# mym-br/gama_tts

Hardware: AMD Instinct MI355X
Metric: audio samples/sec (whole node), batched VTM @44.1kHz (higher is better)
Workload: dtype f32

## Files before the change

### gama_tts_amd/capi.py

```python
import ctypes
import os

import numpy as np

_HERE = os.path.dirname(os.path.abspath(__file__))
_LIB_NAME = "libgama_vtm.so"
N_PARAM = 16
DEVICE_NONE = -1
PRECISION_F64 = 0
PRECISION_MIXED = 1
PRECISION_F32 = 2
TUBE_10_6 = 0
TUBE_30_18 = 1
TABLE_FIR, TABLE_SRC_H, TABLE_SRC_DH, TABLE_WAVETABLE = 0, 1, 2, 3
_STATUS_UNSUPPORTED = 4


class GvtmError(RuntimeError):
    def __init__(self, status, message):
        super().__init__("gvtm status %d: %s" % (status, message))
        self.status = status


class Config(ctypes.Structure):
# ... 171 lines not shown
    if hasattr(L, "gvtm_plan_create_model5_float"):
        L.gvtm_plan_create_model5_float.argtypes = [ctypes.POINTER(Config5), dbl, i32, ctypes.POINTER(vp)]
        L.gvtm_plan_create_model5_float.restype = i32
    L.gvtm_plan_set_timing.argtypes = [vp, i32]
    L.gvtm_plan_set_timing.restype = i32
    L.gvtm_plan_take_kernel_ms.argtypes = [vp, ctypes.POINTER(i32)]
    L.gvtm_plan_take_kernel_ms.restype = dbl
    if diagnostics:
        L.gvtm_debug_set_rows.argtypes = [vp, i32]
        L.gvtm_debug_set_rows.restype = i32
        L.gvtm_debug_set_taps.argtypes = [vp, vp]
        L.gvtm_debug_set_phase_cycles.argtypes = [vp, vp]
        L.gvtm_debug_dpp_selftest.argtypes = [vp, vp]
        L.gvtm_debug_short_math.argtypes = [i32, vp, sz, vp]
        L.gvtm_debug_device_float_math.argtypes = [vp, i32, vp, sz, vp]
        L.gvtm_debug_group_voices.argtypes = [vp, vp, sz, i32, vp, vp, vp, vp]
        L.gvtm_debug_group_voices.restype = i32
    _libs[diagnostics] = L
    return L


def device_count():
    return int(load_library().gvtm_device_count())


class PinnedArray:

    def __init__(self, shape, dtype):
        self._lib = load_library()
        self.array = None
# ... 413 lines not shown
```

### gama_tts_amd/csrc/vtm_capi.cpp

```cpp
#include <hip/hip_runtime.h>

#include <algorithm>
#include <cstdlib>
#include <cstring>
#include <memory>
#include <new>
#include <string>
#include <utility>
#include <vector>

#include "../../include/gama_vtm.h"
#include "vtm_design.hpp"
#include "vtm_kernels.hpp"
#include "vtm_tracks.hpp"
#include "vtm_math.hpp"

namespace {

thread_local std::string g_last_error;

int fail(int status, const std::string& msg)
{
	g_last_error = msg;
	return status;
// ... 73 lines not shown
};

}

#ifndef GVTM_NOISE_TABLE
#define GVTM_NOISE_TABLE 1
#endif

struct gvtm_plan {
	std::vector<gvtm::Design> designs;
	int device = 0;
	int precision = GVTM_PRECISION_F64;
	int rows = 0;
	DeviceBuffer d_wavetable, d_fir, d_src_h, d_src_dh;
	DeviceBuffer d_consts, d_consts5;
	DeviceBuffer d_noise;
	size_t noise_len = 0;
	std::vector<DeviceBuffer> noise_retired;
	struct {
		DeviceBuffer params, frames, audio, counts, maxabs, pcm, scales, voice_ids, groups;
	} host;
	struct {
		DeviceBuffer params, frames, groups;
	} async;
	std::vector<gvtm::TrackConstants> voice_tracks;
	DeviceBuffer d_voice_tracks;
	int compute_units = 0;
	bool timing = false;
	double* debug_taps = nullptr;
	unsigned long long* phase_cycles = nullptr;
// ... 64 lines not shown
	plan->device = device;
	hipDeviceProp_t prop;
	if ((e = hipGetDeviceProperties(&prop, device)) != hipSuccess) return fail_hip(e, "hipGetDeviceProperties");
	if (std::strncmp(prop.gcnArchName, "gfx950", 6) != 0) {
		return fail(GVTM_ERR_NO_DEVICE, std::string("kernels are built for gfx950 only, device is ") + prop.gcnArchName);
	}
	plan->compute_units = prop.multiProcessorCount;
	return GVTM_OK;
}

int upload_tables(gvtm_plan* plan)
{
	const gvtm::Design& dg = plan->designs[0];
	std::vector<gvtm::DeviceConstants> consts;
	std::vector<gvtm::Model5Constants> consts5;
	std::vector<double> wavetables;
	std::vector<float> wavetables_f;
	for (const gvtm::Design& dv : plan->designs) {
		consts.push_back(dv.k);
		if (dg.model5) consts5.push_back(dv.k5);
		wavetables.insert(wavetables.end(), dv.wavetable.begin(), dv.wavetable.end());
		wavetables_f.insert(wavetables_f.end(), dv.wavetable_f.begin(), dv.wavetable_f.end());
	}
	auto upload_design = [&](DeviceBuffer& dst, const std::vector<double>& wide, const std::vector<float>& narrow) {
		return dg.f32 ? upload(dst, narrow) : upload(dst, wide);
	};
	hipError_t e;
	if (!dg.model5) {
		if ((e = upload_design(plan->d_wavetable, wavetables, wavetables_f)) != hipSuccess) return fail_hip(e, "upload wavetable");
		if ((e = upload_design(plan->d_fir, dg.fir, dg.fir_f)) != hipSuccess) return fail_hip(e, "upload fir");
	}
	if ((e = upload_design(plan->d_src_h, dg.src_h, dg.src_h_f)) != hipSuccess) return fail_hip(e, "upload src_h");
	if ((e = upload_design(plan->d_src_dh, dg.src_dh, dg.src_dh_f)) != hipSuccess) return fail_hip(e, "upload src_dh");
	if ((e = upload(plan->d_consts, consts)) != hipSuccess) return fail_hip(e, "upload constants");
	if (dg.model5 && (e = upload(plan->d_consts5, consts5)) != hipSuccess) return fail_hip(e, "upload model 5 constants");
	return GVTM_OK;
}

template <typename Config, typename Differs>
int create_plan(const Config* configs, size_t n_voices, double control_rate, int device, gvtm_plan** plan_out, const char* shared_keys,
		Differs differs, std::string (*design)(const Config&, double, gvtm::Design&))
{
	if (!configs || !plan_out) return fail(GVTM_ERR_INVALID_ARGUMENT, "null config or plan_out");
	*plan_out = nullptr;
	if (n_voices == 0) return fail(GVTM_ERR_INVALID_ARGUMENT, "a plan needs at least one voice");
	if (n_voices > 0x7fffffffu) return fail(GVTM_ERR_INVALID_ARGUMENT, "too many voices");
	for (size_t v = 1; v < n_voices; ++v) {
		if (differs(configs[0], configs[v])) {
			return fail(GVTM_ERR_INVALID_ARGUMENT, "voice " + std::to_string(v) + ": " + shared_keys + " must be those of voice 0 "
					"(one plan is one model at one output rate)");
// ... 269 lines not shown
		case 2: out[i] = gvtm::vmath::cos_short(x[i]); break;
		case 3: out[i] = gvtm::vmath::tan_short(x[i]); break;
		case 4: out[i] = gvtm::vmath::powf_base2(static_cast<float>(x[i])); break;
		case 5: out[i] = gvtm::vmath::powf_base10(static_cast<float>(x[i])); break;
		case 6: out[i] = gvtm::vmath::cosf_glibc(static_cast<float>(x[i])); break;
		case 7: out[i] = gvtm::vmath::tanf_glibc(static_cast<float>(x[i])); break;
		case 8: out[i] = gvtm::vmath::sinf_glibc(static_cast<float>(x[i])); break;
		default: return GVTM_ERR_INVALID_ARGUMENT;
		}
	}
	return GVTM_OK;
}

int gvtm_debug_device_float_math(gvtm_plan* plan, int kind, const float* x, size_t n, float* out)
{
	if (!plan || !x || !out || kind < 0 || kind > 5) return fail(GVTM_ERR_INVALID_ARGUMENT, "bad argument");
	if (plan->device == GVTM_DEVICE_NONE) return fail(GVTM_ERR_NO_DEVICE, "design-only plan");
	DeviceScope scope(plan->device);
	hipError_t e = scope.status();
	if (e != hipSuccess) return fail_hip(e, "hipSetDevice");
	DeviceBuffer dx, dout;
	if ((e = dx.ensure(n * sizeof(float))) != hipSuccess) return fail_hip(e, "hipMalloc");
	if ((e = dout.ensure(n * sizeof(float))) != hipSuccess) return fail_hip(e, "hipMalloc");
	e = hipMemcpy(dx.ptr, x, n * sizeof(float), hipMemcpyHostToDevice);
	if (e == hipSuccess) e = gvtm::launch_float_math_probe(kind, static_cast<const float*>(dx.ptr), n, static_cast<float*>(dout.ptr), nullptr);
	if (e == hipSuccess) e = hipMemcpy(out, dout.ptr, n * sizeof(float), hipMemcpyDeviceToHost);
	if (e != hipSuccess) return fail_hip(e, "float math probe");
	return GVTM_OK;
}

int gvtm_debug_group_voices(gvtm_plan* plan, const int32_t* d_voice_ids, size_t batch, int rows, int32_t* d_row_map, int32_t* d_group_voice,
		int64_t* d_out_counts, float* d_maxabs)
{
	if (!plan || !d_voice_ids || !d_row_map || !d_group_voice || batch == 0 || rows < 1) return fail(GVTM_ERR_INVALID_ARGUMENT, "bad argument");
	if (plan->device == GVTM_DEVICE_NONE) return fail(GVTM_ERR_NO_DEVICE, "design-only plan");
	DeviceScope scope(plan->device);
	hipError_t e = scope.status();
	if (e != hipSuccess) return fail_hip(e, "hipSetDevice");
	DeviceBuffer counts;
	if ((e = counts.ensure(sizeof(int32_t) * plan->n_voices() * gvtm::kGroupVoicesThreads)) != hipSuccess) return fail_hip(e, "hipMalloc");
	const size_t groups = (batch + rows - 1) / rows + static_cast<size_t>(plan->n_voices());
	gvtm::GroupVoicesArgs ga{d_voice_ids, batch, plan->n_voices(), rows, groups, d_row_map, d_group_voice, static_cast<int32_t*>(counts.ptr), d_out_counts, d_maxabs};
// ... 182 lines not shown
	}
	args.src_h = plan->d_src_h.ptr;
	args.src_dh = plan->d_src_dh.ptr;
	args.max_frames = r.max_frames;
	args.audio_stride = r.audio_stride;
	args.batch = r.batch;
	if (r.sl) {
		args.stream = r.sl->d_state;
		args.stream_stride = r.sl->stride;
		args.stream_mode = r.sl->mode;
		if (r.voices && !dg.model5) args.stream_chunk = gvtm::synth_chunk_length(dg.k, plan->precision, 1);
	}
	args.debug_taps = r.voices ? nullptr : plan->debug_taps;
	args.phase_cycles = r.voices ? nullptr : plan->phase_cycles;
	args.k5const = static_cast<const gvtm::Model5Constants*>(plan->d_consts5.ptr);
	return args;
}

template <typename Launch>
int timed_launch(gvtm_plan* plan, hipStream_t stream, const char* what, Launch launch)
{
	hipError_t e;
	EventPair ev;
	if (plan->timing) {
		if (!plan->pool.empty()) {
			ev = std::move(plan->pool.back());
			plan->pool.pop_back();
		} else {
			if ((e = hipEventCreate(&ev.start.h)) != hipSuccess) return fail_hip(e, "hipEventCreate");
			if ((e = hipEventCreate(&ev.stop.h)) != hipSuccess) return fail_hip(e, "hipEventCreate");
// ... 786 lines not shown
```

### gama_tts_amd/csrc/vtm_design.hpp

```cpp
#pragma once

#include <cstddef>
#include <cstdint>
#include <string>
#include <vector>

#include "../../include/gama_vtm.h"

namespace gvtm {

constexpr int kWavetableLength = 512;
constexpr int kSrcZeroCrossings = 13;
constexpr int kSrcPhases = 256;
constexpr int kSrcFilterLength = kSrcZeroCrossings * kSrcPhases;
constexpr int kSrcRing = 1024;
constexpr int kMaxFirTaps = 64;
constexpr int kMaxSectionDelay = 4;
constexpr int kMaxPad = 96;

struct DeviceConstants {
	int sample_rate;
	unsigned control_steps;
	float interp_coef;
	int section_delay;
// ... 9 lines not shown
	double damping;
	double radius_coef[8];
	double aperture_radius2;
	double nasal_r2_sq;
	double nasal_k[6];
	double mouth_b0_refl, mouth_a1_refl, mouth_a_rad;
	double nose_b0_refl, nose_a1_refl, nose_a_rad;
	double throat_b0, throat_a1, throat_gain;
	double bp_T;
	int upsampling;
	int pad;
	unsigned time_inc;
	unsigned phase_inc;
	double src_ratio;
};

struct Model5Constants {
	double sample_rate;
	double output_rate;
	int bypass, constant_mouth;
	double rb_t1, rb_tn_min, rb_tn_max;
	double gn_b0, gn_a1;
	double gp_b0, gp_a1;
	double fn_b0, fn_b1, fn_a1, fn_a2;
	double frication_factor;
	double min_loss, max_loss;
	double nasal_r1_sq;
	double nasal_k[6];
	double period;
	double nose_c[6];
// ... 86 lines not shown
```

### gama_tts_amd/csrc/vtm_device_common.inc

```
#pragma once


constexpr int kDppRowShr1 = 0x111;
constexpr int kDppRowShl1 = 0x101;

__device__ __forceinline__ float from_left(float v)
{
	return __int_as_float(__builtin_amdgcn_update_dpp(0, __float_as_int(v), kDppRowShr1, 0xF, 0xF, true));
}
__device__ __forceinline__ float from_right(float v)
{
	return __int_as_float(__builtin_amdgcn_update_dpp(0, __float_as_int(v), kDppRowShl1, 0xF, 0xF, true));
}
__device__ __forceinline__ double from_left(double v)
{
	const int lo = __builtin_amdgcn_update_dpp(0, __double2loint(v), kDppRowShr1, 0xF, 0xF, true);
	const int hi = __builtin_amdgcn_update_dpp(0, __double2hiint(v), kDppRowShr1, 0xF, 0xF, true);
	return __hiloint2double(hi, lo);
}
__device__ __forceinline__ double from_right(double v)
{
	const int lo = __builtin_amdgcn_update_dpp(0, __double2loint(v), kDppRowShl1, 0xF, 0xF, true);
	const int hi = __builtin_amdgcn_update_dpp(0, __double2hiint(v), kDppRowShl1, 0xF, 0xF, true);
	return __hiloint2double(hi, lo);
// ... 85 lines not shown

__device__ __forceinline__ double frequency_dev(double pitch)
{
	return 220.0 * vmath::exp2_short((pitch + 3.0) * (1.0 / 12.0));
}
__device__ __forceinline__ float frequency_dev(float pitch)
{
	const float x = rmul(pitch + 3.0f, static_cast<float>(1.0 / 12.0));
	return rmul(220.0f, vmath::powf_base2(x));
}

__device__ __forceinline__ double tan_dev(double t) { return vmath::tan_short(t); }
__device__ __forceinline__ double cos_dev(double t) { return vmath::cos_short(t); }
__device__ __forceinline__ float tan_dev(float t) { return vmath::tanf_glibc(t); }
__device__ __forceinline__ float cos_dev(float t) { return vmath::cosf_glibc(t); }

template <typename T> struct Pair;
template <> struct Pair<double> { using type = double2; };
template <> struct Pair<float> { using type = float2; };

__device__ __forceinline__ double noise_advance(double seed)
{
#pragma clang fp contract(off)
	const double product = seed * 377.0;
	return product - floor(product);
}

__device__ __forceinline__ float fdiv_n(float a, float b)
{
	float r = __builtin_amdgcn_rcpf(b);
// ... 50 lines not shown
```

### gama_tts_amd/csrc/vtm_diag_kernels.hip

```cpp
#include <hip/hip_runtime.h>

#include <cstdint>

#include "vtm_design.hpp"
#include "vtm_kernels.hpp"
#include "vtm_math.hpp"

namespace gvtm {

namespace {
#include "vtm_device_common.inc"
}

__global__ void dpp_selftest_kernel(int* out)
{
	const int lane = threadIdx.x & 63;
	const double v = static_cast<double>(lane);
	out[lane] = static_cast<int>(from_left(v));
	out[64 + lane] = static_cast<int>(from_right(v));
	out[128 + lane] = static_cast<int>(row_rotate<6>(v));
	out[192 + lane] = static_cast<int>(row_rotate<10>(v));
	out[256 + lane] = static_cast<int>(from_left_wave(v));
	out[320 + lane] = static_cast<int>(from_right_wave(v));
	out[384 + lane] = static_cast<int>(row_bcast<3>(v));
// ... 3 lines not shown
}


hipError_t launch_dpp_selftest(int* d_out, hipStream_t stream)
{
	hipLaunchKernelGGL(dpp_selftest_kernel, dim3(1), dim3(64), 0, stream, d_out);
	return hipGetLastError();
}

__global__ void float_math_probe_kernel(int kind, const float* x, size_t n, float* out)
{
	const size_t i = static_cast<size_t>(blockIdx.x) * blockDim.x + threadIdx.x;
	if (i >= n) return;
	const float v = x[i];
	float r = 0.0f;
	switch (kind) {
	case 0: r = frequency_dev(v); break;
	case 1: r = amplitude_60db_dev(v); break;
	case 2: r = tan_dev(v); break;
	case 3: r = cos_dev(v); break;
	case 4: r = fdiv_n(v, x[i ^ 1]); break;
	case 5: r = vmath::sinf_glibc(v); break;
	}
	out[i] = r;
}

hipError_t launch_float_math_probe(int kind, const float* d_x, size_t n, float* d_out, hipStream_t stream)
{
	hipLaunchKernelGGL(float_math_probe_kernel, dim3(static_cast<unsigned>((n + 255) / 256)), dim3(256), 0, stream, kind, d_x, n, d_out);
	return hipGetLastError();
// ... 4 lines not shown
```

### gama_tts_amd/csrc/vtm_kernel_v2.inc

```

namespace v2 {

namespace {

constexpr int kPrm = 17;
constexpr int kF1Planes = 6;
constexpr int kF1U = 0, kF1Sig = 1, kF1Thr = 2, kF1B0 = 3, kF1A1 = 4, kF1A2 = 5;
constexpr int kKl = 11;
constexpr int kKlK8 = 7, kKlNk1 = 8, kKlAlr = 9, kKlAu = 10;
constexpr int kInj = 9;
template <typename CT, int LAYOUT>
constexpr bool lane_rec()
{
	return sizeof(CT) == 4 && LAYOUT == 0;
}
constexpr int kLrZero = 16, kLrAlr = 17, kLrAu = 18, kLrK8 = 19, kLrKn = 20, kLrInj = 21, kLrLen = 31;
constexpr int kl_len(bool lr)
{
	return lr ? kLrLen : kKl;
}
template <typename CT>
constexpr bool fr_compact()
{
	return sizeof(CT) == 8;
// ... 405 lines not shown
	__syncthreads();

	if (a.stream) {
		for (int u = 0; u < U; ++u) {
			if (GVTM_ROW_UTT(u, group * U + u) >= a.batch) break;
			const unsigned char* sb = a.stream + GVTM_ROW_UTT(u, (group * U + u)) * a.stream_stride;
			const ST* ring = reinterpret_cast<const ST*>(sb + SL::ring(kTubeLanes, kTubeWords));
			for (int i = tid; i < XRS; i += kThreads) sm.x[u * XRS + i] = ring[i < XR ? i : i - XR];
			const CT* pre = reinterpret_cast<const CT*>(sb + SL::wpre(kTubeLanes, kTubeWords));
			for (int i = tid; i < kWPre; i += kThreads) sm.w[static_cast<size_t>(u) * (kWPre + 2 * C) + i] = pre[i];
		}
		__syncthreads();
	}

	const DeviceConstants& k = *sm.kc;
	int max_chunks = 0;
#pragma unroll
	for (int u = 0; u < U; ++u) max_chunks = sm.ext[u].nchunks > max_chunks ? sm.ext[u].nchunks : max_chunks;

	auto valid_in = [&](int u, int c) -> int {
		const Extent e = sm.ext[u];
		if (c < 0 || c >= e.nchunks) return -1;
		const uint32_t left = e.steps - static_cast<uint32_t>(c) * C;
		return left < static_cast<uint32_t>(C) ? static_cast<int>(left) : C;
	};

	constexpr bool kRowView = !TL::kWaveWide || U > 1;
	const int L = kRowView ? (lane & 15) : lane;
	const int row = kRowView ? (lane >> 4) : 0;
	constexpr bool kTubePerWave = TL::kWaveWide && U > 1;
	constexpr int kFirstHelper = kTubePerWave ? kSerial : 5 * G;
	const int role = kTubePerWave ? (wave < U ? 0 : (wave < kSerial ? wave - U + 1 : 5)) : (wave < 5 * G ? wave / G : 5);
	const int sub = kTubePerWave ? (wave < U ? wave : 0) : (wave < 5 * G ? wave % G : 0);
	const int urow = (U >= 4) ? sub * 4 + row : row % U;
	constexpr int kState = (2 * D + 1) > 5 ? (2 * D + 1) : 5;
	CT st[kState];
#pragma unroll
	for (int i = 0; i < kState; ++i) st[i] = CT(0.0);
	CT& sc_pos = st[0];
// ... 54 lines not shown

	unsigned long long role_busy = 0;
#if GVTM_TUNE_TRACE
	int tr_n = 0;
	auto TR = [&](int t, unsigned id) {
		if (a.phase_cycles != nullptr && group == 0 && lane == 0 && t >= GVTM_TUNE_TRACE && t < GVTM_TUNE_TRACE + 2 && tr_n < 128)
			a.phase_cycles[32768 + wave * 128 + tr_n++] = (static_cast<unsigned long long>(id) << 48) | (clock64() & 0xFFFFFFFFFFFFull);
	};
#else
	auto TR = [](int, unsigned) {};
#endif
	const bool stamping = a.phase_cycles != nullptr && lane == 0;


	auto stage_p2a = [&](int c, int pass) {
		for (int item = pass * 64 + hl; item < U * C && item < (pass + 1) * 64; item += 64) {
			const int u = item / C, s = item - u * C;
			if (s >= valid_in(u, c)) continue;
			const float* pv = sm.prm + at_prm(c & 1, u) + s * kPrm;
			const CT pitch = pv[0], gv = pv[1], av = pv[2];
			const CT f0 = frequency_dev(pitch);
			sm.inc[((c & 1) * U + u) * C + s] = (f0 / CT(2.0)) * CT(k.basic_increment);
			sm.amp[amp_at(c & 3, u, 0, s)] = amplitude_60db_dev(gv);
			sm.amp[amp_at(c & 3, u, 1, s)] = amplitude_60db_dev(av);
		}
	};

	constexpr int kP4aItems = 1;
	auto stage_p4a = [&](int c, int pass) {
		if constexpr (U == 1) {
// ... 51 lines not shown
			const CT v = wl[q] + rmul(p[q] - static_cast<CT>(lower[q]), wu[q] - wl[q]);
			CT* slot = sm.w + (static_cast<size_t>(c % 3) * U + u[q]) * (kWPre + 2 * C);
			slot[kWPre + h[q]] = v;
			if (GVTM_KERNEL_TAPS && a.debug_taps) {
				a.debug_taps[(GVTM_ROW_UTT(u[q], (group * U + u[q])) * a.max_frames * k.control_steps + static_cast<size_t>(c) * C + (h[q] >> 1)) * 8 + 5 + (h[q] & 1)] = p[q];
			}
			if (h[q] >= 2 * C - kWPre) {
				CT* next = sm.w + (static_cast<size_t>((c + 1) % 3) * U + u[q]) * (kWPre + 2 * C);
				next[h[q] - (2 * C - kWPre)] = v;
			}
		}
	};

	auto stage_p4b = [&](int c, int pass) {
		const int taps = k.fir_taps;
		for (int item = pass * 64 + hl; item < U * C && item < (pass + 1) * 64; item += 64) {
			const int u = item / C, s = item - u * C;
			if (s >= valid_in(u, c)) continue;
			CT lp_table = CT(0.0);
			if (kNoiseTable && a.noise_lp != nullptr) lp_table = static_cast<const CT*>(a.noise_lp)[sm.ext[u].step_base + static_cast<unsigned long long>(c) * C + s];
			const CT* wp = sm.w + (static_cast<size_t>(c % 3) * U + u) * (kWPre + 2 * C) + kWPre + 2 * s + 1;
			using CT2 = typename Pair<CT>::type;
			CT acc = 0;
			auto fir_mad = [](CT w, CT cf, CT sum) -> CT {
				if constexpr (sizeof(CT) == 4) return sum + rmul(w, cf);
				else return __builtin_fma(w, cf, sum);
			};
			constexpr int kNT = sizeof(CT) == 8 ? 49 : 47;
			if (sizeof(CT) == 4 && taps == kNT) {
				CT2 wv[kNT / 2];
// ... 33 lines not shown
					}
				}
				}
				for (; i + 1 < taps; i += 2) {
					const CT2 wv = *reinterpret_cast<const CT2*>(wp - i - 1);
					const CT2 cv = *reinterpret_cast<const CT2*>(sm.fir + i);
					acc = fir_mad(wv.y, cv.x, acc);
					acc = fir_mad(wv.x, cv.y, acc);
				}
				if (i < taps) acc = fir_mad(wp[-i], sm.fir[i], acc);
			}
			const CT ax = sm.amp[amp_at(c & 3, u, 0, s)], ah1 = sm.amp[amp_at(c & 3, u, 1, s)];
			const CT lp = (kNoiseTable && a.noise_lp != nullptr) ? lp_table : sm.noise[((c % 3) * U + u) * C + s];
			CT pulse = acc;
			const CT pulsed_noise = rmul(lp, pulse);
			pulse = rmul(ax, rmul(pulse, CT(1.0) - CT(k.breathiness)) + rmul(pulsed_noise, CT(k.breathiness)));
			CT signal;
			if (k.modulation) {
				CT cm = rmul(ax, CT(k.crossmix_factor));
				cm = cm < CT(1.0) ? cm : CT(1.0);
				signal = rmul(pulsed_noise, cm) + rmul(lp, CT(1.0) - cm);
			} else {
				signal = lp;
			}
			CT* usg = sm.usg + at_usg(c & 1, u) + s;
			const CT tube_in = (pulse + rmul(ah1, signal)) * CT(0.125), throat_in = pulse * CT(0.125);
			usg[kF1U * C] = tube_in;
			usg[kF1Sig * C] = signal;
			usg[kF1Thr * C] = throat_in;
			if (GVTM_KERNEL_TAPS && a.debug_taps) {
				double* t = a.debug_taps + (GVTM_ROW_UTT(u, (group * U + u)) * a.max_frames * k.control_steps + static_cast<size_t>(c) * C + s) * 8;
				t[0] = tube_in; t[1] = signal; t[2] = throat_in; t[3] = acc; t[4] = lp;
			}
		}
	};

	auto stage_p2c = [&](int c, int pass) {
		for (int item = pass * 64 + hl; item < U * C && item < (pass + 1) * 64; item += 64) {
			const int u = item / C, s = item - u * C;
			if (s >= valid_in(u, c)) continue;
			const float* pv = sm.prm + at_prm(c & 1, u) + s * kPrm;
			const CT fvol = pv[3], fpos = pv[4], fcf = pv[5], fbw = pv[6];
			CT* fr = sm.fr + at_fr(c & 1, u) + s * kFr;
			const CT amp = amplitude_60db_dev(fvol);
			const int ipart = static_cast<int>(fpos);
			const CT complement = fpos - ipart;
			const CT remainder = CT(1.0) - complement;
			if constexpr (kFrCompact) {
				fr[kFrTapA] = remainder * amp;
				fr[kFrTapB] = complement * amp;
				fr[kFrZero] = CT(0.0);
				*reinterpret_cast<int*>(fr + kFrFirst) = ipart;
// ... 7 lines not shown
				}
				fr[kFr - 1] = CT(0.0);
			}
			const CT pi = CT(3.14159265358979323846);
			const CT tan_v = tan_dev(pi * fbw * CT(k.bp_T));
			const CT cos_v = cos_dev(CT(2.0) * pi * fcf * CT(k.bp_T));
			const CT a2 = (CT(1.0) - tan_v) / (CT(1.0) + tan_v);
			CT* bpc = sm.usg + at_usg(c & 1, u) + s;
			bpc[kF1B0 * C] = CT(0.5) - rmul(CT(0.5), a2);
			bpc[kF1A1 * C] = -(CT(1.0) + a2) * cos_v;
			bpc[kF1A2 * C] = a2;
		}
	};

	auto stage_p2b = [&](int c, int pass) {
		for (int item = pass * 64 + hl; item < U * C && item < (pass + 1) * 64; item += 64) {
			const int u = item / C, s = item - u * C;
			if (s >= valid_in(u, c)) continue;
			const float* cur = sm.prm + at_prm(c & 1, u) + s * kPrm + 7;
			CT r2[8];
#pragma unroll
			for (int q = 0; q < 8; ++q) {
				CT r = static_cast<CT>(cur[q]) * CT(k.radius_coef[q]);
				r = r > CT(0.01) ? r : CT(0.01);
				r2[q] = rmul(r, r);
			}
			const CT velum2 = rmul(static_cast<CT>(cur[8]), static_cast<CT>(cur[8]));
			CT kj[8];
#pragma unroll
			for (int q = 0; q < 7; ++q) kj[q] = fdiv_n(r2[q] - r2[q + 1], r2[q] + r2[q + 1]);
			kj[7] = fdiv_n(r2[7] - CT(k.aperture_radius2), r2[7] + CT(k.aperture_radius2));
			const CT asum = fdiv_n(CT(2.0), r2[3] + r2[3] + velum2);
			const CT nk1 = fdiv_n(velum2 - CT(k.nasal_r2_sq), velum2 + CT(k.nasal_r2_sq));
			CT* kl = sm.kl + at_kl(c & 1, u) + (kLaneRec ? 0 : s * kKlLen);
			if constexpr (kLaneRec) {
#pragma unroll
				for (int Lq = 0; Lq < 16; ++Lq) {
					const int q = TL::lane(Lq).kl_slot;
					if (q >= 0) kl[kl_index(s, Lq)] = (q == kKlNk1) ? nk1 : kj[q < 7 ? q : 0];
				}
				kl[kl_index(s, kLrAlr)] = asum * r2[3];
				kl[kl_index(s, kLrAu)] = asum * velum2;
				kl[kl_index(s, kLrK8)] = kj[7];
				sm.opk[((c % 3) * U + u) * C + s] = CT(1.0) + kj[7];
			} else {
#pragma unroll
				for (int q = 0; q < 7; ++q) kl[q] = kj[q];
				kl[kKlK8] = kj[7];
// ... 969 lines not shown
```

### gama_tts_amd/csrc/vtm_kernels.hpp

```cpp
#pragma once

#include <hip/hip_runtime.h>

#include <cstddef>
#include <cstdint>

#include "vtm_design.hpp"

namespace gvtm {

struct StreamHeader {
	unsigned long long step_base;
	double seed;
	unsigned peak_bits;
	unsigned reserved_;
	unsigned long long pad_;
};
static_assert(sizeof(StreamHeader) == 32, "stream header layout");
constexpr int kStreamScalars = 12;
constexpr int kSsPos = 0, kSsPrev = 1;
constexpr int kSsBp = 2, kSsThr = 6;
constexpr int kSsRadMouth = 7, kSsRadNose = 9;
constexpr int kStreamPreRoll = 48;
enum StreamMode : int { kStreamNone = 0, kStreamPush = 1, kStreamFinish = 2 };
// ... 39 lines not shown
	const void* noise_lp = nullptr;
	unsigned long long noise_len = 0;
	size_t max_frames;
	size_t audio_stride;
	size_t batch;
	int xr;
	unsigned char* stream = nullptr;
	size_t stream_stride = 0;
	int stream_mode = kStreamNone;
	double* debug_taps;
	unsigned long long* phase_cycles;
	const Model5Constants* k5const = nullptr;
	const int32_t* row_map = nullptr;
	const int32_t* group_voice = nullptr;
	int stream_chunk = 0;
};

struct GroupVoicesArgs {
	const int32_t* voice_ids;
	size_t batch;
	int n_voices;
	int rows;
	size_t groups;
	int32_t* row_map;
	int32_t* group_voice;
	int32_t* counts;
	int64_t* out_counts;
	float* maxabs;
};
constexpr int kGroupVoicesThreads = 256;
// ... 36 lines not shown
```

### gama_tts_amd/csrc/vtm_math.hpp

```cpp
#pragma once

#include <cmath>
#include <cstdint>
#include <cstring>

#if defined(__HIPCC__)
#define GVTM_HD __host__ __device__ __forceinline__
#else
#define GVTM_HD inline
#endif

namespace gvtm {
namespace vmath {

GVTM_HD double exp_small(double t)
{
	double p = 1.0 / 6227020800.0;
	p = std::fma(p, t, 1.0 / 479001600.0);
	p = std::fma(p, t, 1.0 / 39916800.0);
	p = std::fma(p, t, 1.0 / 3628800.0);
	p = std::fma(p, t, 1.0 / 362880.0);
	p = std::fma(p, t, 1.0 / 40320.0);
	p = std::fma(p, t, 1.0 / 5040.0);
	p = std::fma(p, t, 1.0 / 720.0);
// ... 75 lines not shown
	const double k = std::rint(t * 0.63661977236758134308);
	const double r = reduce_half_pi(t, k);
	if (k == 0.0) return cos_kernel(r);
	if (k == 1.0) return -sin_kernel(r);
	return -cos_kernel(r);
}

GVTM_HD double tan_short(double t)
{
	if (!(t >= 0.0 && t < 1.5)) return std::tan(t);
	if (t <= 0.78539816339744830962) return sin_kernel(t) / cos_kernel(t);
	const double r = -reduce_half_pi(t, 1.0);
	return cos_kernel(r) / sin_kernel(r);
}

GVTM_HD float powf_exp2_core(double xd)
{
#if defined(__clang__)
#pragma clang fp contract(off)
#endif
	constexpr uint64_t tab[32] = {
		0x3ff0000000000000ull, 0x3fefd9b0d3158574ull, 0x3fefb5586cf9890full, 0x3fef9301d0125b51ull,
		0x3fef72b83c7d517bull, 0x3fef54873168b9aaull, 0x3fef387a6e756238ull, 0x3fef1e9df51fdee1ull,
		0x3fef06fe0a31b715ull, 0x3feef1a7373aa9cbull, 0x3feedea64c123422ull, 0x3feece086061892dull,
		0x3feebfdad5362a27ull, 0x3feeb42b569d4f82ull, 0x3feeab07dd485429ull, 0x3feea47eb03a5585ull,
		0x3feea09e667f3bcdull, 0x3fee9f75e8ec5f74ull, 0x3feea11473eb0187ull, 0x3feea589994cce13ull,
		0x3feeace5422aa0dbull, 0x3feeb737b0cdc5e5ull, 0x3feec49182a3f090ull, 0x3feed503b23e255dull,
		0x3feee89f995ad3adull, 0x3feeff76f2fb5e47ull, 0x3fef199bdd85529cull, 0x3fef3720dcef9069ull,
		0x3fef5818dcfba487ull, 0x3fef7c97337b9b5full, 0x3fefa4afa2a490daull, 0x3fefd0765b6e4540ull};
	constexpr double c0 = 0x1.c6af84b912394p-5, c1 = 0x1.ebfce50fac4f3p-3, c2 = 0x1.62e42ff0c52d6p-1;
	constexpr double shift = 0x1.8p+52 / 32;
	double kd = xd + shift;
	uint64_t ki;
	std::memcpy(&ki, &kd, sizeof(ki));
	kd -= shift;
	const double r = xd - kd;
	const uint64_t t = tab[ki & 31u] + (ki << 47);
	double s;
	std::memcpy(&s, &t, sizeof(s));
	const double z = c0 * r + c1;
	const double r2 = r * r;
	double y = c2 * r + 1.0;
	y = z * r2 + y;
	y = y * s;
	return static_cast<float>(y);
}

GVTM_HD float powf_base2(float x)
{
	if (!(std::fabs(x) < 100.0f)) return static_cast<float>(std::exp2(static_cast<double>(x)));
	return powf_exp2_core(static_cast<double>(x));
}

GVTM_HD float powf_base10(float y)
{
#if defined(__clang__)
#pragma clang fp contract(off)
#endif
	if (!(std::fabs(y) < 30.0f)) return static_cast<float>(std::pow(10.0, static_cast<double>(y)));
	constexpr double log2_10_glibc = 0x1.a934f0979b22dp+1;
	const double ylogx = static_cast<double>(y) * log2_10_glibc;
	return powf_exp2_core(ylogx);
}

GVTM_HD uint32_t float_bits(float f)
{
	uint32_t u;
	std::memcpy(&u, &f, sizeof(u));
	return u;
}
GVTM_HD float bits_float(uint32_t u)
{
	float f;
	std::memcpy(&f, &u, sizeof(f));
	return f;
}

GVTM_HD float cosf_glibc(float y)
{
#if defined(__clang__)
#pragma clang fp contract(off)
#endif
	const uint32_t top = (float_bits(y) >> 20) & 0x7ffu;
	if (!(top < ((float_bits(120.0f) >> 20) & 0x7ffu))) return static_cast<float>(std::cos(static_cast<double>(y)));
	constexpr double hpi_inv = 0x1.45F306DC9C883p+23, hpi = 0x1.921FB54442D18p0;
	constexpr double c0 = 0x1p0, c1 = -0x1.ffffffd0c621cp-2, c2 = 0x1.55553e1068f19p-5, c3 = -0x1.6c087e89a359dp-10,
			c4 = 0x1.99343027bf8c3p-16;
	constexpr double s1 = -0x1.555545995a603p-3, s2 = 0x1.1107605230bc4p-7, s3 = -0x1.994eb3774cf24p-13;
	double x = y;
	int n = 1;
	double flip = 1.0;
	if (top < ((float_bits(0x1.921FB6p-1f) >> 20) & 0x7ffu)) {
		if (top < ((float_bits(0x1p-12f) >> 20) & 0x7ffu)) return 1.0f;
	} else {
		const double r = x * hpi_inv;
		const int q = (static_cast<int32_t>(r) + 0x800000) >> 24;
		x = x - q * hpi;
		const double sgn = ((q & 3) == 1 || (q & 3) == 2) ? -1.0 : 1.0;
		if (q & 2) flip = -1.0;
// ... 11 lines not shown
		const double d2 = flip * c3 + x2r * (flip * c4);
		const double d1 = flip * c0 + x2r * (flip * c1);
		const double x6 = x4 * x2r;
		const double d = d1 + x4 * (flip * c2);
		return static_cast<float>(d + x6 * d2);
	}
	const double x2 = x * x;
	const double x4 = x2 * x2;
	const double d2 = c3 + x2 * c4;
	const double d1 = c0 + x2 * c1;
	const double x6 = x4 * x2;
	const double d = d1 + x4 * c2;
	return static_cast<float>(d + x6 * d2);
}

GVTM_HD float sinf_glibc(float y)
{
#if defined(__clang__)
#pragma clang fp contract(off)
#endif
	const uint32_t top = (float_bits(y) >> 20) & 0x7ffu;
	if (!(top < ((float_bits(120.0f) >> 20) & 0x7ffu))) return static_cast<float>(std::sin(static_cast<double>(y)));
	constexpr double hpi_inv = 0x1.45F306DC9C883p+23, hpi = 0x1.921FB54442D18p0;
	constexpr double c0 = 0x1p0, c1 = -0x1.ffffffd0c621cp-2, c2 = 0x1.55553e1068f19p-5, c3 = -0x1.6c087e89a359dp-10,
			c4 = 0x1.99343027bf8c3p-16;
	constexpr double s1 = -0x1.555545995a603p-3, s2 = 0x1.1107605230bc4p-7, s3 = -0x1.994eb3774cf24p-13;
	double x = y;
	double x2 = x * x;
	int n = 0;
	double flip = 1.0;
// ... 58 lines not shown
	r += T0 * s;
	w = x + r;
	if (big) {
		v = static_cast<float>(iy);
		return v - 2.0f * (x - (w * w / (w + v) - r));
	}
	if (iy == 1) return w;
	z = bits_float(float_bits(w) & 0xfffff000u);
	v = r - (z - x);
	const float a = -1.0f / w;
	const float t = bits_float(float_bits(a) & 0xfffff000u);
	s = 1.0f + t * z;
	return t + a * (s + t * v);
}

GVTM_HD float tanf_glibc(float x)
{
#if defined(__clang__)
#pragma clang fp contract(off)
#endif
	if (!(x >= 0.0f && x <= 1.38f)) return static_cast<float>(std::tan(static_cast<double>(x)));
	const uint32_t ix = float_bits(x);
	if (ix <= 0x3f490fdau) return tanf_kernel_glibc(x, 0.0f, 1);
	constexpr float pio2_1 = 1.5707855225e+00f, pio2_1t = 1.0804334124e-05f, pio2_2 = 1.0804273188e-05f,
			pio2_2t = 6.0770999344e-11f;
	float z = x - pio2_1, y0, y1;
	if ((ix & 0xfffffff0u) != 0x3fc90fd0u) {
		y0 = z - pio2_1t;
		y1 = (z - y0) - pio2_1t;
	} else {
		z -= pio2_2;
		y0 = z - pio2_2t;
		y1 = (z - y0) - pio2_2t;
	}
	const float m = tanf_kernel_glibc(-y0, -y1, -1);
	return -m;
}

}
}
```

Baseline: 15.79 billion.

## Use float constant block and wave-held exp2 table in f32 parameter stages

Adds a per-voice FloatConstants block in constant address space so the f32 stages read pre-narrowed scalars instead of converting doubles. The exp2 table is held one entry per lane and looked up with ds_bpermute rather than indexed from a constant array. Range checks for powf, tan and cos move to a wave-uniform cold path behind __any with noinline fallbacks. The p2a/p2c stages drop their per-item loop for a single branch-free item per lane, aiming to cut scalar/vector register pressure and divergence. This adds complexity, and results must stay bit-identical with the previous glibc-matching math.

```diff
diff --git a/gama_tts_amd/capi.py b/gama_tts_amd/capi.py
--- a/gama_tts_amd/capi.py
+++ b/gama_tts_amd/capi.py
@@ -209,6 +209,8 @@
         L.gvtm_debug_dpp_selftest.argtypes = [vp, vp]
         L.gvtm_debug_short_math.argtypes = [i32, vp, sz, vp]
         L.gvtm_debug_device_float_math.argtypes = [vp, i32, vp, sz, vp]
+        L.gvtm_debug_float_constants.argtypes = [vp, i32, vp, vp]
+        L.gvtm_debug_float_constants.restype = i32
         L.gvtm_debug_group_voices.argtypes = [vp, vp, sz, i32, vp, vp, vp, vp]
         L.gvtm_debug_group_voices.restype = i32
     _libs[diagnostics] = L
diff --git a/gama_tts_amd/csrc/vtm_capi.cpp b/gama_tts_amd/csrc/vtm_capi.cpp
--- a/gama_tts_amd/csrc/vtm_capi.cpp
+++ b/gama_tts_amd/csrc/vtm_capi.cpp
@@ -111,6 +111,7 @@
 	int rows = 0;
 	DeviceBuffer d_wavetable, d_fir, d_src_h, d_src_dh;
 	DeviceBuffer d_consts, d_consts5;
+	DeviceBuffer d_consts_f;
 	DeviceBuffer d_noise;
 	size_t noise_len = 0;
 	std::vector<DeviceBuffer> noise_retired;
@@ -205,11 +206,13 @@
 	const gvtm::Design& dg = plan->designs[0];
 	std::vector<gvtm::DeviceConstants> consts;
 	std::vector<gvtm::Model5Constants> consts5;
+	std::vector<gvtm::FloatConstants> consts_f;
 	std::vector<double> wavetables;
 	std::vector<float> wavetables_f;
 	for (const gvtm::Design& dv : plan->designs) {
 		consts.push_back(dv.k);
 		if (dg.model5) consts5.push_back(dv.k5);
+		else if (dg.f32) consts_f.push_back(gvtm::float_constants(dv.k));
 		wavetables.insert(wavetables.end(), dv.wavetable.begin(), dv.wavetable.end());
 		wavetables_f.insert(wavetables_f.end(), dv.wavetable_f.begin(), dv.wavetable_f.end());
 	}
@@ -225,6 +228,7 @@
 	if ((e = upload_design(plan->d_src_dh, dg.src_dh, dg.src_dh_f)) != hipSuccess) return fail_hip(e, "upload src_dh");
 	if ((e = upload(plan->d_consts, consts)) != hipSuccess) return fail_hip(e, "upload constants");
 	if (dg.model5 && (e = upload(plan->d_consts5, consts5)) != hipSuccess) return fail_hip(e, "upload model 5 constants");
+	if (!consts_f.empty() && (e = upload(plan->d_consts_f, consts_f)) != hipSuccess) return fail_hip(e, "upload float constants");
 	return GVTM_OK;
 }
 
@@ -524,7 +528,7 @@
 
 int gvtm_debug_device_float_math(gvtm_plan* plan, int kind, const float* x, size_t n, float* out)
 {
-	if (!plan || !x || !out || kind < 0 || kind > 5) return fail(GVTM_ERR_INVALID_ARGUMENT, "bad argument");
+	if (!plan || !x || !out || kind < 0 || kind > 11 || (kind >= 6 && n % 64 != 0)) return fail(GVTM_ERR_INVALID_ARGUMENT, "bad argument");
 	if (plan->device == GVTM_DEVICE_NONE) return fail(GVTM_ERR_NO_DEVICE, "design-only plan");
 	DeviceScope scope(plan->device);
 	hipError_t e = scope.status();
@@ -536,6 +540,26 @@
 	if (e == hipSuccess) e = gvtm::launch_float_math_probe(kind, static_cast<const float*>(dx.ptr), n, static_cast<float*>(dout.ptr), nullptr);
 	if (e == hipSuccess) e = hipMemcpy(out, dout.ptr, n * sizeof(float), hipMemcpyDeviceToHost);
 	if (e != hipSuccess) return fail_hip(e, "float math probe");
+	return GVTM_OK;
+}
+
+int gvtm_debug_float_constants(gvtm_plan* plan, int voice, void* block64, double* fields15)
+{
+	if (!plan || !block64 || !fields15 || voice < 0 || voice >= plan->n_voices()) return fail(GVTM_ERR_INVALID_ARGUMENT, "bad argument");
+	if (plan->designs[0].model5 || !plan->designs[0].f32) return fail(GVTM_ERR_UNSUPPORTED, "float plans of models 0 to 4 only");
+	const gvtm::DeviceConstants& k = plan->designs[voice].k;
+	const gvtm::FloatConstants f = gvtm::float_constants(k);
+	static_assert(sizeof(f) == 64, "FloatConstants: 15 floats and one integer");
+	std::memcpy(block64, &f, sizeof(f));
+	int n = 0;
+	fields15[n++] = k.basic_increment;
+	fields15[n++] = k.breathiness;
+	fields15[n++] = 1.0 - k.breathiness;
+	fields15[n++] = k.crossmix_factor;
+	for (int q = 0; q < 8; ++q) fields15[n++] = k.radius_coef[q];
+	fields15[n++] = k.aperture_radius2;
+	fields15[n++] = k.nasal_r2_sq;
+	fields15[n++] = k.bp_T;
 	return GVTM_OK;
 }
 
@@ -748,6 +772,7 @@
 	args.debug_taps = r.voices ? nullptr : plan->debug_taps;
 	args.phase_cycles = r.voices ? nullptr : plan->phase_cycles;
 	args.k5const = static_cast<const gvtm::Model5Constants*>(plan->d_consts5.ptr);
+	args.kfconst = static_cast<const gvtm::FloatConstants*>(plan->d_consts_f.ptr);
 	return args;
 }
 
diff --git a/gama_tts_amd/csrc/vtm_design.hpp b/gama_tts_amd/csrc/vtm_design.hpp
--- a/gama_tts_amd/csrc/vtm_design.hpp
+++ b/gama_tts_amd/csrc/vtm_design.hpp
@@ -47,6 +47,33 @@
 	unsigned phase_inc;
 	double src_ratio;
 };
+
+struct FloatConstants {
+	float basic_increment;
+	float breathiness;
+	float one_minus_breathiness;
+	float crossmix_factor;
+	float radius_coef[8];
+	float aperture_radius2;
+	float nasal_r2_sq;
+	float bp_T;
+	int modulation;
+};
+
+inline FloatConstants float_constants(const DeviceConstants& k)
+{
+	FloatConstants f{};
+	f.basic_increment = static_cast<float>(k.basic_increment);
+	f.breathiness = static_cast<float>(k.breathiness);
+	f.one_minus_breathiness = 1.0f - f.breathiness;
+	f.crossmix_factor = static_cast<float>(k.crossmix_factor);
+	for (int q = 0; q < 8; ++q) f.radius_coef[q] = static_cast<float>(k.radius_coef[q]);
+	f.aperture_radius2 = static_cast<float>(k.aperture_radius2);
+	f.nasal_r2_sq = static_cast<float>(k.nasal_r2_sq);
+	f.bp_T = static_cast<float>(k.bp_T);
+	f.modulation = k.modulation;
+	return f;
+}
 
 struct Model5Constants {
 	double sample_rate;
diff --git a/gama_tts_amd/csrc/vtm_device_common.inc b/gama_tts_amd/csrc/vtm_device_common.inc
--- a/gama_tts_amd/csrc/vtm_device_common.inc
+++ b/gama_tts_amd/csrc/vtm_device_common.inc
@@ -123,6 +123,71 @@
 __device__ __forceinline__ double cos_dev(double t) { return vmath::cos_short(t); }
 __device__ __forceinline__ float tan_dev(float t) { return vmath::tanf_glibc(t); }
 __device__ __forceinline__ float cos_dev(float t) { return vmath::cosf_glibc(t); }
+
+__device__ __forceinline__ uint64_t powf_tab_hold(int lane)
+{
+	return vmath::powf_exp2_tab(static_cast<unsigned>(lane) & 31u);
+}
+__device__ __forceinline__ uint64_t powf_tab_lookup(uint64_t held, uint64_t ki)
+{
+	const int src = static_cast<int>(static_cast<unsigned>(ki) & 31u) << 2;
+	const unsigned lo = static_cast<unsigned>(__builtin_amdgcn_ds_bpermute(src, static_cast<int>(static_cast<unsigned>(held))));
+	const unsigned hi = static_cast<unsigned>(__builtin_amdgcn_ds_bpermute(src, static_cast<int>(static_cast<unsigned>(held >> 32))));
+	return (static_cast<uint64_t>(hi) << 32) | lo;
+}
+[[maybe_unused]] __device__ __noinline__ float powf_base2_cold(float x) { return static_cast<float>(std::exp2(static_cast<double>(x))); }
+[[maybe_unused]] __device__ __noinline__ float powf_base10_cold(float y) { return static_cast<float>(std::pow(10.0, static_cast<double>(y))); }
+[[maybe_unused]] __device__ __noinline__ float tanf_cold(float x) { return static_cast<float>(std::tan(static_cast<double>(x))); }
+[[maybe_unused]] __device__ __noinline__ float cosf_cold(float x) { return static_cast<float>(std::cos(static_cast<double>(x))); }
+
+__device__ __forceinline__ bool amplitude_uses_powf(float db) { return !(db <= 0.0f) && !(db == 60.0f); }
+__device__ __forceinline__ float amplitude_select(float db, float p) { return db <= 0.0f ? 0.0f : (db == 60.0f ? 1.0f : p); }
+
+__device__ __forceinline__ void p2a_convert(float pitch, float gv, float av, uint64_t held, float& f0, float& ax, float& ah1)
+{
+	const float x = rmul(pitch + 3.0f, static_cast<float>(1.0 / 12.0));
+	const float yg = rmul(gv - 60.0f, static_cast<float>(1.0 / 20.0));
+	const float ya = rmul(av - 60.0f, static_cast<float>(1.0 / 20.0));
+	uint64_t kx, kg, ka;
+	const double rx = vmath::powf_exp2_split(static_cast<double>(x), kx);
+	const double rg = vmath::powf_exp2_split(vmath::powf_ylog2_10(yg), kg);
+	const double ra = vmath::powf_exp2_split(vmath::powf_ylog2_10(ya), ka);
+	const uint64_t ex = powf_tab_lookup(held, kx), eg = powf_tab_lookup(held, kg), ea = powf_tab_lookup(held, ka);
+	float px = vmath::powf_exp2_poly(rx, kx, ex);
+	float pg = vmath::powf_exp2_poly(rg, kg, eg);
+	float pa = vmath::powf_exp2_poly(ra, ka, ea);
+	const bool cx = !(fabsf(x) < 100.0f);
+	const bool cg = amplitude_uses_powf(gv) && !(fabsf(yg) < 30.0f);
+	const bool ca = amplitude_uses_powf(av) && !(fabsf(ya) < 30.0f);
+	if (__any(cx || cg || ca)) {
+		if (cx) px = powf_base2_cold(x);
+		if (cg) pg = powf_base10_cold(yg);
+		if (ca) pa = powf_base10_cold(ya);
+	}
+	f0 = rmul(220.0f, px);
+	ax = amplitude_select(gv, pg);
+	ah1 = amplitude_select(av, pa);
+}
+
+__device__ __forceinline__ void p2c_convert(float fvol, float tan_arg, float cos_arg, uint64_t held, float& amp, float& tan_v, float& cos_v)
+{
+	const float y = rmul(fvol - 60.0f, static_cast<float>(1.0 / 20.0));
+	uint64_t ky;
+	const double ry = vmath::powf_exp2_split(vmath::powf_ylog2_10(y), ky);
+	const uint64_t ey = powf_tab_lookup(held, ky);
+	float p = vmath::powf_exp2_poly(ry, ky, ey);
+	tan_v = vmath::tanf_glibc_core(tan_arg);
+	cos_v = vmath::cosf_glibc_core(cos_arg);
+	const bool cy = amplitude_uses_powf(fvol) && !(fabsf(y) < 30.0f);
+	const bool ct = !vmath::tanf_glibc_in_range(tan_arg);
+	const bool cc = !vmath::cosf_glibc_in_range(cos_arg);
+	if (__any(cy || ct || cc)) {
+		if (cy) p = powf_base10_cold(y);
+		if (ct) tan_v = tanf_cold(tan_arg);
+		if (cc) cos_v = cosf_cold(cos_arg);
+	}
+	amp = amplitude_select(fvol, p);
+}
 
 template <typename T> struct Pair;
 template <> struct Pair<double> { using type = double2; };
diff --git a/gama_tts_amd/csrc/vtm_diag_kernels.hip b/gama_tts_amd/csrc/vtm_diag_kernels.hip
--- a/gama_tts_amd/csrc/vtm_diag_kernels.hip
+++ b/gama_tts_amd/csrc/vtm_diag_kernels.hip
@@ -41,6 +41,19 @@
 	if (i >= n) return;
 	const float v = x[i];
 	float r = 0.0f;
+	if (kind >= 6) {
+		const uint64_t held = powf_tab_hold(static_cast<int>(threadIdx.x & 63));
+		float p0, p1, p2;
+		if (kind <= 8) {
+			p2a_convert(kind == 6 ? v : -12.0f, kind == 7 ? v : 54.0f, kind == 8 ? v : 0.0f, held, p0, p1, p2);
+			r = kind == 6 ? p0 : (kind == 7 ? p1 : p2);
+		} else {
+			p2c_convert(kind == 9 ? v : 25.0f, kind == 10 ? v : 0.07f, kind == 11 ? v : 0.4f, held, p0, p1, p2);
+			r = kind == 9 ? p0 : (kind == 10 ? p1 : p2);
+		}
+		out[i] = r;
+		return;
+	}
 	switch (kind) {
 	case 0: r = frequency_dev(v); break;
 	case 1: r = amplitude_60db_dev(v); break;
diff --git a/gama_tts_amd/csrc/vtm_kernel_v2.inc b/gama_tts_amd/csrc/vtm_kernel_v2.inc
--- a/gama_tts_amd/csrc/vtm_kernel_v2.inc
+++ b/gama_tts_amd/csrc/vtm_kernel_v2.inc
@@ -443,6 +443,17 @@
 	}
 
 	const DeviceConstants& k = *sm.kc;
+	using KF = const __attribute__((address_space(4))) FloatConstants;
+	[[maybe_unused]] auto float_consts = [&]() -> KF* {
+		KF* p = (KF*)(a.kfconst + voice);
+		asm volatile("" : "+s"(p));
+		return p;
+	};
+	[[maybe_unused]] auto fresh_lane = [&]() -> int {
+		int l = hl;
+		asm volatile("" : "+v"(l));
+		return l;
+	};
 	int max_chunks = 0;
 #pragma unroll
 	for (int u = 0; u < U; ++u) max_chunks = sm.ext[u].nchunks > max_chunks ? sm.ext[u].nchunks : max_chunks;
@@ -452,6 +463,11 @@
 		if (c < 0 || c >= e.nchunks) return -1;
 		const uint32_t left = e.steps - static_cast<uint32_t>(c) * C;
 		return left < static_cast<uint32_t>(C) ? static_cast<int>(left) : C;
+	};
+	[[maybe_unused]] auto valid_of = [](const Extent& e, int c) -> int {
+		const uint32_t left = e.steps - static_cast<uint32_t>(c) * C;
+		const int v = left < static_cast<uint32_t>(C) ? static_cast<int>(left) : C;
+		return (c < 0 || c >= e.nchunks) ? -1 : v;
 	};
 
 	constexpr bool kRowView = !TL::kWaveWide || U > 1;
@@ -536,6 +552,24 @@
 
 
 	auto stage_p2a = [&](int c, int pass) {
+		if constexpr (sizeof(CT) == 4) {
+			KF* const kf = float_consts();
+			const float binc = kf->basic_increment;
+			const uint64_t held = powf_tab_hold(fresh_lane());
+			const int item = pass * 64 + hl;
+			const int uq = item / C, u = uq < U ? uq : U - 1, s = item - uq * C;
+			const Extent e = sm.ext[u];
+			const float* pv = sm.prm + at_prm(c & 1, u) + s * kPrm;
+			const float pitch = pv[0], gv = pv[1], av = pv[2];
+			float f0, ax, ah1;
+			p2a_convert(pitch, gv, av, held, f0, ax, ah1);
+			if (uq < U && s < valid_of(e, c)) {
+				sm.inc[((c & 1) * U + u) * C + s] = (f0 / 2.0f) * binc;
+				sm.amp[amp_at(c & 3, u, 0, s)] = ax;
+				sm.amp[amp_at(c & 3, u, 1, s)] = ah1;
+			}
+			return;
+		}
 		for (int item = pass * 64 + hl; item < U * C && item < (pass + 1) * 64; item += 64) {
 			const int u = item / C, s = item - u * C;
 			if (s >= valid_in(u, c)) continue;
@@ -617,6 +651,29 @@
 
 	auto stage_p4b = [&](int c, int pass) {
 		const int taps = k.fir_taps;
+		[[maybe_unused]] float kf_breath = 0.0f, kf_omb = 0.0f, kf_crossmix = 0.0f;
+		[[maybe_unused]] int kf_modulation = 0;
+		if constexpr (sizeof(CT) == 4) {
+			KF* const kf = float_consts();
+			kf_breath = kf->breathiness; kf_omb = kf->one_minus_breathiness; kf_crossmix = kf->crossmix_factor;
+			kf_modulation = kf->modulation;
+		}
+		auto breathiness = [&]() -> CT {
+			if constexpr (sizeof(CT) == 4) return kf_breath;
+			else return CT(k.breathiness);
+		};
+		auto one_minus_breathiness = [&]() -> CT {
+			if constexpr (sizeof(CT) == 4) return kf_omb;
+			else return CT(1.0) - CT(k.breathiness);
+		};
+		auto crossmix_factor = [&]() -> CT {
+			if constexpr (sizeof(CT) == 4) return kf_crossmix;
+			else return CT(k.crossmix_factor);
+		};
+		auto modulation = [&]() -> int {
+			if constexpr (sizeof(CT) == 4) return kf_modulation;
+			else return k.modulation;
+		};
 		for (int item = pass * 64 + hl; item < U * C && item < (pass + 1) * 64; item += 64) {
 			const int u = item / C, s = item - u * C;
 			if (s >= valid_in(u, c)) continue;
@@ -680,10 +737,10 @@
 			const CT lp = (kNoiseTable && a.noise_lp != nullptr) ? lp_table : sm.noise[((c % 3) * U + u) * C + s];
 			CT pulse = acc;
 			const CT pulsed_noise = rmul(lp, pulse);
-			pulse = rmul(ax, rmul(pulse, CT(1.0) - CT(k.breathiness)) + rmul(pulsed_noise, CT(k.breathiness)));
+			pulse = rmul(ax, rmul(pulse, one_minus_breathiness()) + rmul(pulsed_noise, breathiness()));
 			CT signal;
-			if (k.modulation) {
-				CT cm = rmul(ax, CT(k.crossmix_factor));
+			if (modulation()) {
+				CT cm = rmul(ax, crossmix_factor());
 				cm = cm < CT(1.0) ? cm : CT(1.0);
 				signal = rmul(pulsed_noise, cm) + rmul(lp, CT(1.0) - cm);
 			} else {
@@ -702,6 +759,45 @@
 	};
 
 	auto stage_p2c = [&](int c, int pass) {
+		if constexpr (sizeof(CT) == 4) {
+			KF* const kf = float_consts();
+			const float bp_T = kf->bp_T;
+			const uint64_t held = powf_tab_hold(fresh_lane());
+			const int item = pass * 64 + hl;
+			const int uq = item / C, u = uq < U ? uq : U - 1, s = item - uq * C;
+			const Extent e = sm.ext[u];
+			const float* pv = sm.prm + at_prm(c & 1, u) + s * kPrm;
+			const float fvol = pv[3], fpos = pv[4], fcf = pv[5], fbw = pv[6];
+			const float pi = 3.14159265358979323846f;
+			float amp, tan_v, cos_v;
+			p2c_convert(fvol, pi * fbw * bp_T, 2.0f * pi * fcf * bp_T, held, amp, tan_v, cos_v);
+			if (!(uq < U && s < valid_of(e, c))) return;
+			float* fr = sm.fr + at_fr(c & 1, u) + s * kFr;
+			const int ipart = static_cast<int>(fpos);
+			const float complement = fpos - ipart;
+			const float remainder = 1.0f - complement;
+			if constexpr (kFrCompact) {
+				fr[kFrTapA] = remainder * amp;
+				fr[kFrTapB] = complement * amp;
+				fr[kFrZero] = 0.0f;
+				*reinterpret_cast<int*>(fr + kFrFirst) = ipart;
+			} else {
+#pragma unroll
+				for (int q = 0; q < 8; ++q) {
+					float t = 0.0f;
+					if (q == ipart) t = remainder * amp;
+					else if (q == ipart + 1) t = complement * amp;
+					fr[q] = t;
+				}
+				fr[kFr - 1] = 0.0f;
+			}
+			const float a2 = (1.0f - tan_v) / (1.0f + tan_v);
+			float* bpc = sm.usg + at_usg(c & 1, u) + s;
+			bpc[kF1B0 * C] = 0.5f - rmul(0.5f, a2);
+			bpc[kF1A1 * C] = -(1.0f + a2) * cos_v;
+			bpc[kF1A2 * C] = a2;
+			return;
+		}
 		for (int item = pass * 64 + hl; item < U * C && item < (pass + 1) * 64; item += 64) {
 			const int u = item / C, s = item - u * C;
 			if (s >= valid_in(u, c)) continue;
@@ -739,24 +835,57 @@
 	};
 
 	auto stage_p2b = [&](int c, int pass) {
+		[[maybe_unused]] float kf_rc[8], kf_ap = 0.0f, kf_nr = 0.0f;
+		if constexpr (sizeof(CT) == 4) {
+			KF* const kf = float_consts();
+#pragma unroll
+			for (int q = 0; q < 8; ++q) kf_rc[q] = kf->radius_coef[q];
+			kf_ap = kf->aperture_radius2;
+			kf_nr = kf->nasal_r2_sq;
+		}
+		auto radius_coef = [&](int q) -> CT {
+			if constexpr (sizeof(CT) == 4) return kf_rc[q];
+			else return CT(k.radius_coef[q]);
+		};
+		auto aperture_radius2 = [&]() -> CT {
+			if constexpr (sizeof(CT) == 4) return kf_ap;
+			else return CT(k.aperture_radius2);
+		};
+		auto nasal_r2_sq = [&]() -> CT {
+			if constexpr (sizeof(CT) == 4) return kf_nr;
+			else return CT(k.nasal_r2_sq);
+		};
 		for (int item = pass * 64 + hl; item < U * C && item < (pass + 1) * 64; item += 64) {
 			const int u = item / C, s = item - u * C;
-			if (s >= valid_in(u, c)) continue;
+			[[maybe_unused]] float curv[9];
+			if constexpr (sizeof(CT) == 4) {
+				const Extent e = sm.ext[u];
+				const float* curp = sm.prm + at_prm(c & 1, u) + s * kPrm + 7;
+#pragma unroll
+				for (int q = 0; q < 9; ++q) curv[q] = curp[q];
+				if (s >= valid_of(e, c)) continue;
+			} else {
+				if (s >= valid_in(u, c)) continue;
+			}
 			const float* cur = sm.prm + at_prm(c & 1, u) + s * kPrm + 7;
+			auto cur_at = [&](int q) -> float {
+				if constexpr (sizeof(CT) == 4) return curv[q];
+				else return cur[q];
+			};
 			CT r2[8];
 #pragma unroll
 			for (int q = 0; q < 8; ++q) {
-				CT r = static_cast<CT>(cur[q]) * CT(k.radius_coef[q]);
+				CT r = static_cast<CT>(cur_at(q)) * radius_coef(q);
 				r = r > CT(0.01) ? r : CT(0.01);
 				r2[q] = rmul(r, r);
 			}
-			const CT velum2 = rmul(static_cast<CT>(cur[8]), static_cast<CT>(cur[8]));
+			const CT velum2 = rmul(static_cast<CT>(cur_at(8)), static_cast<CT>(cur_at(8)));
 			CT kj[8];
 #pragma unroll
 			for (int q = 0; q < 7; ++q) kj[q] = fdiv_n(r2[q] - r2[q + 1], r2[q] + r2[q + 1]);
-			kj[7] = fdiv_n(r2[7] - CT(k.aperture_radius2), r2[7] + CT(k.aperture_radius2));
+			kj[7] = fdiv_n(r2[7] - aperture_radius2(), r2[7] + aperture_radius2());
 			const CT asum = fdiv_n(CT(2.0), r2[3] + r2[3] + velum2);
-			const CT nk1 = fdiv_n(velum2 - CT(k.nasal_r2_sq), velum2 + CT(k.nasal_r2_sq));
+			const CT nk1 = fdiv_n(velum2 - nasal_r2_sq(), velum2 + nasal_r2_sq());
 			CT* kl = sm.kl + at_kl(c & 1, u) + (kLaneRec ? 0 : s * kKlLen);
 			if constexpr (kLaneRec) {
 #pragma unroll
diff --git a/gama_tts_amd/csrc/vtm_kernels.hpp b/gama_tts_amd/csrc/vtm_kernels.hpp
--- a/gama_tts_amd/csrc/vtm_kernels.hpp
+++ b/gama_tts_amd/csrc/vtm_kernels.hpp
@@ -77,6 +77,7 @@
 	const int32_t* row_map = nullptr;
 	const int32_t* group_voice = nullptr;
 	int stream_chunk = 0;
+	const FloatConstants* kfconst = nullptr;
 };
 
 struct GroupVoicesArgs {
diff --git a/gama_tts_amd/csrc/vtm_math.hpp b/gama_tts_amd/csrc/vtm_math.hpp
--- a/gama_tts_amd/csrc/vtm_math.hpp
+++ b/gama_tts_amd/csrc/vtm_math.hpp
@@ -113,11 +113,8 @@
 	return cos_kernel(r) / sin_kernel(r);
 }
 
-GVTM_HD float powf_exp2_core(double xd)
-{
-#if defined(__clang__)
-#pragma clang fp contract(off)
-#endif
+GVTM_HD uint64_t powf_exp2_tab(unsigned i)
+{
 	constexpr uint64_t tab[32] = {
 		0x3ff0000000000000ull, 0x3fefd9b0d3158574ull, 0x3fefb5586cf9890full, 0x3fef9301d0125b51ull,
 		0x3fef72b83c7d517bull, 0x3fef54873168b9aaull, 0x3fef387a6e756238ull, 0x3fef1e9df51fdee1ull,
@@ -127,14 +124,27 @@
 		0x3feeace5422aa0dbull, 0x3feeb737b0cdc5e5ull, 0x3feec49182a3f090ull, 0x3feed503b23e255dull,
 		0x3feee89f995ad3adull, 0x3feeff76f2fb5e47ull, 0x3fef199bdd85529cull, 0x3fef3720dcef9069ull,
 		0x3fef5818dcfba487ull, 0x3fef7c97337b9b5full, 0x3fefa4afa2a490daull, 0x3fefd0765b6e4540ull};
-	constexpr double c0 = 0x1.c6af84b912394p-5, c1 = 0x1.ebfce50fac4f3p-3, c2 = 0x1.62e42ff0c52d6p-1;
+	return tab[i];
+}
+
+GVTM_HD double powf_exp2_split(double xd, uint64_t& ki)
+{
+#if defined(__clang__)
+#pragma clang fp contract(off)
+#endif
 	constexpr double shift = 0x1.8p+52 / 32;
 	double kd = xd + shift;
-	uint64_t ki;
 	std::memcpy(&ki, &kd, sizeof(ki));
 	kd -= shift;
-	const double r = xd - kd;
-	const uint64_t t = tab[ki & 31u] + (ki << 47);
+	return xd - kd;
+}
+GVTM_HD float powf_exp2_poly(double r, uint64_t ki, uint64_t entry)
+{
+#if defined(__clang__)
+#pragma clang fp contract(off)
+#endif
+	constexpr double c0 = 0x1.c6af84b912394p-5, c1 = 0x1.ebfce50fac4f3p-3, c2 = 0x1.62e42ff0c52d6p-1;
+	const uint64_t t = entry + (ki << 47);
 	double s;
 	std::memcpy(&s, &t, sizeof(s));
 	const double z = c0 * r + c1;
@@ -144,6 +154,12 @@
 	y = y * s;
 	return static_cast<float>(y);
 }
+GVTM_HD float powf_exp2_core(double xd)
+{
+	uint64_t ki;
+	const double r = powf_exp2_split(xd, ki);
+	return powf_exp2_poly(r, ki, powf_exp2_tab(static_cast<unsigned>(ki & 31u)));
+}
 
 GVTM_HD float powf_base2(float x)
 {
@@ -151,15 +167,22 @@
 	return powf_exp2_core(static_cast<double>(x));
 }
 
+GVTM_HD double powf_ylog2_10(float y)
+{
+#if defined(__clang__)
+#pragma clang fp contract(off)
+#endif
+	constexpr double log2_10_glibc = 0x1.a934f0979b22dp+1;
+	return static_cast<double>(y) * log2_10_glibc;
+}
+
 GVTM_HD float powf_base10(float y)
 {
 #if defined(__clang__)
 #pragma clang fp contract(off)
 #endif
 	if (!(std::fabs(y) < 30.0f)) return static_cast<float>(std::pow(10.0, static_cast<double>(y)));
-	constexpr double log2_10_glibc = 0x1.a934f0979b22dp+1;
-	const double ylogx = static_cast<double>(y) * log2_10_glibc;
-	return powf_exp2_core(ylogx);
+	return powf_exp2_core(powf_ylog2_10(y));
 }
 
 GVTM_HD uint32_t float_bits(float f)
@@ -175,13 +198,17 @@
 	return f;
 }
 
-GVTM_HD float cosf_glibc(float y)
+GVTM_HD bool cosf_glibc_in_range(float y)
+{
+	return ((float_bits(y) >> 20) & 0x7ffu) < ((float_bits(120.0f) >> 20) & 0x7ffu);
+}
+
+GVTM_HD float cosf_glibc_core(float y)
 {
 #if defined(__clang__)
 #pragma clang fp contract(off)
 #endif
 	const uint32_t top = (float_bits(y) >> 20) & 0x7ffu;
-	if (!(top < ((float_bits(120.0f) >> 20) & 0x7ffu))) return static_cast<float>(std::cos(static_cast<double>(y)));
 	constexpr double hpi_inv = 0x1.45F306DC9C883p+23, hpi = 0x1.921FB54442D18p0;
 	constexpr double c0 = 0x1p0, c1 = -0x1.ffffffd0c621cp-2, c2 = 0x1.55553e1068f19p-5, c3 = -0x1.6c087e89a359dp-10,
 			c4 = 0x1.99343027bf8c3p-16;
@@ -223,6 +250,12 @@
 	return static_cast<float>(d + x6 * d2);
 }
 
+GVTM_HD float cosf_glibc(float y)
+{
+	if (!cosf_glibc_in_range(y)) return static_cast<float>(std::cos(static_cast<double>(y)));
+	return cosf_glibc_core(y);
+}
+
 GVTM_HD float sinf_glibc(float y)
 {
 #if defined(__clang__)
@@ -311,12 +344,16 @@
 	return t + a * (s + t * v);
 }
 
-GVTM_HD float tanf_glibc(float x)
-{
-#if defined(__clang__)
-#pragma clang fp contract(off)
-#endif
-	if (!(x >= 0.0f && x <= 1.38f)) return static_cast<float>(std::tan(static_cast<double>(x)));
+GVTM_HD bool tanf_glibc_in_range(float x)
+{
+	return x >= 0.0f && x <= 1.38f;
+}
+
+GVTM_HD float tanf_glibc_core(float x)
+{
+#if defined(__clang__)
+#pragma clang fp contract(off)
+#endif
 	const uint32_t ix = float_bits(x);
 	if (ix <= 0x3f490fdau) return tanf_kernel_glibc(x, 0.0f, 1);
 	constexpr float pio2_1 = 1.5707855225e+00f, pio2_1t = 1.0804334124e-05f, pio2_2 = 1.0804273188e-05f,
@@ -334,5 +371,11 @@
 	return -m;
 }
 
-}
-}
+GVTM_HD float tanf_glibc(float x)
+{
+	if (!tanf_glibc_in_range(x)) return static_cast<float>(std::tan(static_cast<double>(x)));
+	return tanf_glibc_core(x);
+}
+
+}
+}
```

Result: no change. 15.87 billion, median of 6 (+0.5%).
